# google/speedy

Hardware: AMD Instinct MI355X
Metric: Msamples/s processed (16 kHz mono, 3.5x nonlinear) (higher is better)
Workload: dtype int16 samples; f64 DFT, f32 features, int32 AMDF/OLA

## Files before the change

### include/speedy_hip.h

```cpp
#ifndef SPEEDY_HIP_H_
#define SPEEDY_HIP_H_
#include <stddef.h>
#include <stdint.h>
#ifdef __cplusplus
extern "C" {
#endif

#ifndef SPX_FEATURE_COUNT
#define SPX_FEATURE_COUNT 15
#endif

typedef struct spx_plan* spx_plan_t;

typedef struct {
  int64_t in_off;
  int64_t n_in;
  int64_t out_off;
  int64_t out_cap;
  int32_t channels;
  float speed;
  float nonlinear;
  float feedback;
} spx_stream_job;

// ... 63 lines not shown
int64_t spx_pipeline_submit(spx_pipeline_t p, const int16_t* in, int in_is_device);
int64_t spx_pipeline_submit_jobs(spx_pipeline_t p, const spx_stream_job* jobs, const int16_t* in, int in_is_device);
int spx_pipeline_jobs_fit(spx_pipeline_t p, const spx_stream_job* jobs);
int spx_pipeline_input_consumed(spx_pipeline_t p, int64_t ticket);
int spx_pipeline_wait(spx_pipeline_t p, int64_t ticket, const int16_t** out, const int64_t** offsets, const int64_t** counts);

float* spx_pipeline_host_input_float(spx_pipeline_t p);
int64_t spx_pipeline_submit_float(spx_pipeline_t p, const float* in, int in_is_device);
int64_t spx_pipeline_submit_jobs_float(spx_pipeline_t p, const spx_stream_job* jobs, const float* in, int in_is_device);
int spx_pipeline_wait_float(spx_pipeline_t p, int64_t ticket, const float** out, const int64_t** offsets, const int64_t** counts);

void* spx_host_alloc(size_t bytes);
void spx_host_free(void* p);

int spx_batch_analyze(spx_plan_t plan, const spx_stream_job* jobs, int n_streams, const int16_t* in,
                      void* workspace, size_t workspace_bytes, const spx_taps* taps, void* hip_stream);
int spx_batch_walk(spx_plan_t plan, const spx_stream_job* jobs, int n_streams, const int16_t* in,
                   int16_t* out, int64_t* n_out, void* workspace, size_t workspace_bytes,
                   const spx_taps* taps, void* hip_stream);

size_t spx_batch_workspace_bytes_mixed(const spx_plan_t* plans, int n_plans, const spx_stream_job* jobs,
                                       const int* plan_index, int n_streams);
int spx_batch_run_mixed(const spx_plan_t* plans, int n_plans, const spx_stream_job* jobs, const int* plan_index,
                        int n_streams, const int16_t* in, int16_t* out, int64_t* n_out, void* workspace,
                        size_t workspace_bytes, void* hip_stream);

int spx_batch_run_mixed_taps(const spx_plan_t* plans, int n_plans, const spx_stream_job* jobs, const int* plan_index,
                             int n_streams, const int16_t* in, int16_t* out, int64_t* n_out, void* workspace,
                             size_t workspace_bytes, const spx_taps* taps, void* hip_stream);
int spx_batch_run_mixed_ahead(const spx_plan_t* plans, int n_plans, const spx_stream_job* jobs, const int* plan_index,
                              int n_streams, const int16_t* in, int16_t* out, int64_t* n_out, void* workspace,
                              size_t workspace_bytes, void* hip_stream);

void spx_set_timing(int enabled);
void spx_set_pipeline_chunks(int chunks);
void spx_set_concurrent(int on);
int spx_timing_collect(double* sum_ms_analyze, double* sum_ms_walk, int* n_calls);
const char* spx_batch_kernel_names(spx_plan_t plan, int n_streams, int max_channels, int speedup_only);
const char* spx_batch_kernel_names_lean(spx_plan_t plan, int n_streams, int max_channels, int speedup_only);
int spx_debug_last_walk_form(void);
int spx_debug_kernel_vgprs(int which);
int spx_debug_walk_info(int sample_rate, int channels, int n_streams, int speedup_only, int short_jobs, int lean, int* out5);
int spx_debug_analysis_info(int sample_rate, int* out4);
int spx_debug_lane_consts(int sample_rate, void* out, double* tw, double* tw2, float* win);
int spx_debug_mode_resources(int sample_rate, int channels, int n_streams, int speedup_only, long long* out22);
long long spx_debug_fdiv_check(unsigned seed, unsigned denominators, int exp_lo, int exp_hi);
long long spx_debug_xfade_check(int n_lo, int n_hi);
long long spx_debug_arith_check(unsigned seed, unsigned threads, unsigned per_thread);
int spx_debug_select_check(const unsigned* d, int n_vectors, int p0, int n_lags, int max_period, int two_per_lane, int* lag_index,
                           unsigned* kmin);
int spx_debug_select_fold_check(const unsigned* d, int n_vectors, int p0, int n_lags, int want_max, int fresh, int* out3);
int spx_debug_log_check(unsigned first_block, unsigned end_block, unsigned long long* sums);
int spx_debug_last_call_concurrent(void);
double spx_timing_last_tension_ms(void);
double spx_timing_last_rate_ms(void);

int spx_batch_read_steps(spx_plan_t plan, const spx_stream_job* jobs, int n_streams, const void* workspace,
                         int32_t* steps, void* hip_stream);
int spx_batch_read_steps_mixed(const spx_plan_t* plans, int n_plans, const spx_stream_job* jobs, const int* plan_index,
                               int n_streams, const void* workspace, int32_t* steps, void* hip_stream);

void* spx_device_alloc(size_t bytes);
void spx_device_free(void* p);
int spx_batch_pack_outputs(const spx_stream_job* jobs, int n_streams, const int16_t* out, const int64_t* n_out,
                           int16_t* packed, int64_t* offsets, void* hip_stream);
int spx_copy_to_device(void* dst, const void* src, size_t bytes, void* hip_stream);
int spx_copy_to_host(void* dst, const void* src, size_t bytes, void* hip_stream);
int spx_stream_synchronize(void* hip_stream);

#ifdef __cplusplus
}
#endif
#endif
```

### speedy_amd/_lib.py

```python
import ctypes as C
import os
import subprocess

_HERE = os.path.dirname(os.path.abspath(__file__))
LIB_PATH = os.environ.get("SPEEDY_HIP_LIB") or os.path.join(_HERE, "lib", "libspeedy_hip.so")
_LIB = None

c_short_p = C.POINTER(C.c_short)
c_float_p = C.POINTER(C.c_float)
c_int64_p = C.POINTER(C.c_int64)


class StreamJob(C.Structure):
    _fields_ = [("in_off", C.c_int64), ("n_in", C.c_int64), ("out_off", C.c_int64), ("out_cap", C.c_int64),
                ("channels", C.c_int32), ("speed", C.c_float), ("nonlinear", C.c_float), ("feedback", C.c_float)]


class Taps(C.Structure):
    _fields_ = [("tension", C.c_void_p), ("speed", C.c_void_p), ("features", C.c_void_p),
                ("spectrogram", C.c_void_p), ("normalized", C.c_void_p)]


TENSION_FN = C.CFUNCTYPE(None, C.c_void_p, C.c_int, C.c_float)
FEATURES_FN = C.CFUNCTYPE(None, C.c_void_p, C.c_int, c_float_p)
# ... 4 lines not shown
    "spx_plan_create": (C.c_void_p, [C.c_int, C.c_int]),
    "spx_plan_destroy": (None, [C.c_void_p]),
    "spx_plan_frame_step": (C.c_int, [C.c_void_p]),
    "spx_plan_window_size": (C.c_int, [C.c_void_p]),
    "spx_plan_fft_size": (C.c_int, [C.c_void_p]),
    "spx_plan_future": (C.c_int, [C.c_void_p]),
    "spx_plan_max_required": (C.c_int, [C.c_void_p]),
    "spx_plan_frames": (C.c_int64, [C.c_void_p, C.c_int64]),
    "spx_plan_out_capacity": (C.c_int64, [C.c_void_p, C.c_int64, C.c_float]),
    "spx_plan_out_capacity_for": (C.c_int64, [C.c_void_p, C.c_int64, C.c_float, C.c_float]),
    "spx_batch_workspace_bytes": (C.c_size_t, [C.c_void_p, C.POINTER(StreamJob), C.c_int]),
    "spx_batch_run": (C.c_int, [C.c_void_p, C.POINTER(StreamJob), C.c_int, C.c_void_p, C.c_void_p, C.c_void_p,
                                C.c_void_p, C.c_size_t, C.POINTER(Taps), C.c_void_p]),
    "spx_batch_run_rate": (C.c_int, [C.c_void_p, C.POINTER(StreamJob), c_float_p, C.c_int, C.c_void_p, C.c_void_p, C.c_void_p,
                                     C.c_void_p, C.c_size_t, C.POINTER(Taps), C.c_void_p]),
    "spx_batch_workspace_bytes_rate": (C.c_size_t, [C.c_void_p, C.POINTER(StreamJob), c_float_p, C.c_int]),
    "spx_plan_out_capacity_rate": (C.c_int64, [C.c_void_p, C.c_int64, C.c_float, C.c_float, C.c_float]),
    "spx_batch_workspace_bytes_float": (C.c_size_t, [C.c_void_p, C.POINTER(StreamJob), c_float_p, C.c_int]),
    "spx_batch_run_float": (C.c_int, [C.c_void_p, C.POINTER(StreamJob), c_float_p, C.c_int, C.c_void_p, C.c_void_p, C.c_void_p,
                                      C.c_void_p, C.c_size_t, C.POINTER(Taps), C.c_void_p]),
    "spx_float_to_short": (C.c_int, [C.c_void_p, C.c_void_p, C.c_size_t, C.c_int, C.c_void_p]),
    "spx_short_to_float": (C.c_int, [C.c_void_p, C.c_void_p, C.c_size_t, C.c_void_p]),
    "spx_batch_run_ahead": (C.c_int, [C.c_void_p, C.POINTER(StreamJob), C.c_int, C.c_void_p, C.c_void_p, C.c_void_p,
                                      C.c_void_p, C.c_size_t, C.POINTER(Taps), C.c_void_p]),
    "spx_batch_run_overlapped": (C.c_int, [C.c_void_p, C.POINTER(StreamJob), C.c_int, C.c_void_p, C.c_void_p, C.c_void_p,
                                           C.c_void_p, C.c_size_t, C.POINTER(Taps), C.c_void_p]),
    "spx_batch_run_ahead_when": (C.c_int, [C.c_void_p, C.POINTER(StreamJob), C.c_int, C.c_void_p, C.c_void_p, C.c_void_p,
                                           C.c_void_p, C.c_size_t, C.POINTER(Taps), C.c_void_p, C.c_void_p]),
    "spx_batch_workspace_bytes_mixed": (C.c_size_t, [C.POINTER(C.c_void_p), C.c_int, C.POINTER(StreamJob), C.POINTER(C.c_int), C.c_int]),
    "spx_batch_run_mixed": (C.c_int, [C.POINTER(C.c_void_p), C.c_int, C.POINTER(StreamJob), C.POINTER(C.c_int), C.c_int,
                                      C.c_void_p, C.c_void_p, C.c_void_p, C.c_void_p, C.c_size_t, C.c_void_p]),
    "spx_batch_run_mixed_ahead": (C.c_int, [C.POINTER(C.c_void_p), C.c_int, C.POINTER(StreamJob), C.POINTER(C.c_int), C.c_int,
                                      C.c_void_p, C.c_void_p, C.c_void_p, C.c_void_p, C.c_size_t, C.c_void_p]),
    "spx_batch_run_mixed_taps": (C.c_int, [C.POINTER(C.c_void_p), C.c_int, C.POINTER(StreamJob), C.POINTER(C.c_int), C.c_int,
                                           C.c_void_p, C.c_void_p, C.c_void_p, C.c_void_p, C.c_size_t, C.POINTER(Taps), C.c_void_p]),
    "spx_batch_read_steps": (C.c_int, [C.c_void_p, C.POINTER(StreamJob), C.c_int, C.c_void_p, C.POINTER(C.c_int32), C.c_void_p]),
    "spx_batch_read_steps_mixed": (C.c_int, [C.POINTER(C.c_void_p), C.c_int, C.POINTER(StreamJob), C.POINTER(C.c_int), C.c_int,
                                             C.c_void_p, C.POINTER(C.c_int32), C.c_void_p]),
    "spx_batch_analyze": (C.c_int, [C.c_void_p, C.POINTER(StreamJob), C.c_int, C.c_void_p, C.c_void_p,
                                    C.c_size_t, C.POINTER(Taps), C.c_void_p]),
    "spx_batch_walk": (C.c_int, [C.c_void_p, C.POINTER(StreamJob), C.c_int, C.c_void_p, C.c_void_p, C.c_void_p,
                                 C.c_void_p, C.c_size_t, C.POINTER(Taps), C.c_void_p]),
    "spx_set_timing": (None, [C.c_int]),
    "spx_set_pipeline_chunks": (None, [C.c_int]),
    "spx_set_concurrent": (None, [C.c_int]),
    "spx_timing_collect": (C.c_int, [C.POINTER(C.c_double), C.POINTER(C.c_double), C.POINTER(C.c_int)]),
    "spx_timing_last_tension_ms": (C.c_double, []),
    "spx_timing_last_rate_ms": (C.c_double, []),
    "spx_batch_kernel_names": (C.c_char_p, [C.c_void_p, C.c_int, C.c_int, C.c_int]),
    "spx_batch_kernel_names_lean": (C.c_char_p, [C.c_void_p, C.c_int, C.c_int, C.c_int]),
    "spx_debug_last_walk_form": (C.c_int, []),
    "spx_debug_kernel_vgprs": (C.c_int, [C.c_int]),
    "spx_debug_last_call_concurrent": (C.c_int, []),
    "spx_debug_fdiv_check": (C.c_longlong, [C.c_uint, C.c_uint, C.c_int, C.c_int]),
    "spx_debug_xfade_check": (C.c_longlong, [C.c_int, C.c_int]),
    "spx_debug_select_check": (C.c_int, [C.POINTER(C.c_uint), C.c_int, C.c_int, C.c_int, C.c_int, C.c_int, C.POINTER(C.c_int), C.POINTER(C.c_uint)]),
    "spx_debug_select_fold_check": (C.c_int, [C.POINTER(C.c_uint), C.c_int, C.c_int, C.c_int, C.c_int, C.c_int, C.POINTER(C.c_int)]),
    "spx_debug_arith_check": (C.c_longlong, [C.c_uint, C.c_uint, C.c_uint]),
    "spx_debug_log_check": (C.c_int, [C.c_uint, C.c_uint, C.POINTER(C.c_ulonglong)]),
    "spx_debug_walk_info": (C.c_int, [C.c_int, C.c_int, C.c_int, C.c_int, C.c_int, C.c_int, C.POINTER(C.c_int)]),
    "spx_debug_analysis_info": (C.c_int, [C.c_int, C.POINTER(C.c_int)]),
    "spx_debug_lane_consts": (C.c_int, [C.c_int, C.c_void_p, C.POINTER(C.c_double), C.POINTER(C.c_double), c_float_p]),
    "spx_debug_mode_resources": (C.c_int, [C.c_int, C.c_int, C.c_int, C.c_int, C.POINTER(C.c_longlong)]),
    "spx_pipeline_create": (C.c_void_p, [C.c_void_p, C.POINTER(StreamJob), C.c_int, C.c_int, C.c_uint]),
    "spx_pipeline_create_mixed": (C.c_void_p, [C.POINTER(C.c_void_p), C.c_int, C.POINTER(StreamJob), C.POINTER(C.c_int), C.c_int, C.c_int, C.c_uint]),
    "spx_pipeline_destroy": (None, [C.c_void_p]),
    "spx_pipeline_depth": (C.c_int, [C.c_void_p]),
    "spx_pipeline_input_values": (C.c_size_t, [C.c_void_p]),
    "spx_pipeline_host_input": (C.c_void_p, [C.c_void_p]),
    "spx_pipeline_submit": (C.c_int64, [C.c_void_p, C.c_void_p, C.c_int]),
    "spx_pipeline_submit_jobs": (C.c_int64, [C.c_void_p, C.POINTER(StreamJob), C.c_void_p, C.c_int]),
    "spx_pipeline_jobs_fit": (C.c_int, [C.c_void_p, C.POINTER(StreamJob)]),
    "spx_pipeline_input_consumed": (C.c_int, [C.c_void_p, C.c_int64]),
    "spx_pipeline_wait": (C.c_int, [C.c_void_p, C.c_int64, C.POINTER(C.c_void_p), C.POINTER(C.c_void_p), C.POINTER(C.c_void_p)]),
    "spx_pipeline_host_input_float": (C.c_void_p, [C.c_void_p]),
    "spx_pipeline_submit_float": (C.c_int64, [C.c_void_p, C.c_void_p, C.c_int]),
    "spx_pipeline_submit_jobs_float": (C.c_int64, [C.c_void_p, C.POINTER(StreamJob), C.c_void_p, C.c_int]),
    "spx_pipeline_wait_float": (C.c_int, [C.c_void_p, C.c_int64, C.POINTER(C.c_void_p), C.POINTER(C.c_void_p), C.POINTER(C.c_void_p)]),
    "spx_host_alloc": (C.c_void_p, [C.c_size_t]),
    "spx_host_free": (None, [C.c_void_p]),
    "spx_device_alloc": (C.c_void_p, [C.c_size_t]),
    "spx_device_free": (None, [C.c_void_p]),
    "spx_copy_to_device": (C.c_int, [C.c_void_p, C.c_void_p, C.c_size_t, C.c_void_p]),
    "spx_copy_to_host": (C.c_int, [C.c_void_p, C.c_void_p, C.c_size_t, C.c_void_p]),
    "spx_batch_pack_outputs": (C.c_int, [C.c_void_p, C.c_int, C.c_void_p, C.c_void_p, C.c_void_p, C.c_void_p, C.c_void_p]),
    "spx_stream_synchronize": (C.c_int, [C.c_void_p]),
    "sonicCreateStream": (C.c_void_p, [C.c_int, C.c_int]),
    "sonicDestroyStream": (None, [C.c_void_p]),
    "sonicWriteShortToStream": (C.c_int, [C.c_void_p, c_short_p, C.c_int]),
    "sonicReadShortFromStream": (C.c_int, [C.c_void_p, c_short_p, C.c_int]),
    "sonicWriteFloatToStream": (C.c_int, [C.c_void_p, c_float_p, C.c_int]),
    "sonicReadFloatFromStream": (C.c_int, [C.c_void_p, c_float_p, C.c_int]),
    "sonicSetRate": (None, [C.c_void_p, C.c_float]),
    "sonicSetSpeed": (None, [C.c_void_p, C.c_float]),
    "sonicFlushStream": (C.c_int, [C.c_void_p]),
    "sonicEnableNonlinearSpeedup": (None, [C.c_void_p, C.c_float]),
    "sonicSetDurationFeedbackStrength": (None, [C.c_void_p, C.c_float]),
    "getSonicBufferSize": (C.c_int, [C.c_void_p]),
    "sonicSpectrogramSize": (C.c_int, [C.c_void_p]),
    "sonicTensionCallback": (None, [C.c_void_p, TENSION_FN]),
    "getSonicTensionCallback": (C.c_void_p, [C.c_void_p]),
    "sonicSpeedCallback": (None, [C.c_void_p, TENSION_FN]),
    "getSonicSpeedCallback": (C.c_void_p, [C.c_void_p]),
    "sonicFeaturesCallback": (None, [C.c_void_p, FEATURES_FN]),
    "getSonicFeaturesCallback": (C.c_void_p, [C.c_void_p]),
    "sonicSpectrogramCallback": (None, [C.c_void_p, FEATURES_FN]),
# ... 86 lines not shown
```

### speedy_amd/csrc/speedy_api.hip

```cpp
#include <math.h>
#include <string.h>

#include <algorithm>
#include <string>
#include <vector>

#include "../../include/speedy.h"
#include "spx_internal.h"
#include "spx_log.h"

extern "C" const char* speedyHipLastError(void);
void spx_internal_set_api_error(const std::string& msg);
int spx_internal_match_matlab();

#define SPD_KEEP 24

struct speedyStreamStruct {
  const SpxPlanDev* plan = nullptr;
  int device = 0, rate = 0;
  hipStream_t hs = nullptr;
  int64_t origin = 0, cap = 0;
  float* dFrames = nullptr;
  SpxFrameRec* dRec = nullptr;
  float* dScr = nullptr;
// ... 34 lines not shown
                 {reinterpret_cast<void**>(&s->tTension), sizeof(float), 1, nullptr},
                 {reinterpret_cast<void**>(&s->tSpeed), sizeof(float), 1, nullptr},
                 {reinterpret_cast<void**>(&s->tFeatures), sizeof(float), SPX_FEATURE_COUNT, nullptr},
                 {reinterpret_cast<void**>(&s->tSpec), sizeof(float), P.N, nullptr},
                 {reinterpret_cast<void**>(&s->tNorm), sizeof(float), P.W, nullptr}};
  for (Arr& a : arrs) {
    if (hipMallocAsync(&a.np, (size_t)ncap * a.stride * a.elem, s->hs) != hipSuccess) {
      (void)hipGetLastError();
      for (Arr& b : arrs) if (b.np) (void)hipFreeAsync(b.np, s->hs);
      return false;
    }
  }
  for (Arr& a : arrs) {
    unsigned char* np = static_cast<unsigned char*>(a.np);
    unsigned char* op = static_cast<unsigned char*>(*a.p);
    const size_t row = (size_t)a.stride * a.elem;
    (void)hipMemsetAsync(np, 0, (size_t)ncap * row, s->hs);
    if (op && keep_hi > keep_lo) {
      const int64_t n = std::min(keep_hi, s->origin + s->cap) - keep_lo;
      if (n > 0)
        (void)hipMemcpyAsync(np + (size_t)(keep_lo - lo) * row, op + (size_t)(keep_lo - s->origin) * row, (size_t)n * row,
                             hipMemcpyDeviceToDevice, s->hs);
    }
    if (op) (void)hipFreeAsync(op, s->hs);
    *a.p = a.np;
  }
  s->origin = lo;
  s->cap = ncap;
  return true;
}

static bool launch(speedyStream s, bool new_frame, int64_t k_from, int64_t k_to) {
  const SpxPlanDev& P = *s->plan;
  if (!grow(s, s->T + 2)) { spx_internal_set_api_error("speedy: device allocation failed"); return false; }
  SpxStreamDev J;
  memset(&J, 0, sizeof(J));
  J.frame_off = -s->origin;
  J.n_frames = (int32_t)(s->T + (new_frame ? 1 : 0));
  J.frame_begin = (int32_t)s->T;
  J.channels = 1;
  J.flags = (s->started ? 0 : SPX_F_INIT) | SPX_F_TENSION_RANGE | SPX_F_NO_SPEED;
  J.speed = 2.0f; J.nonlinear = 1.0f; J.feedback = 0.0f;
  J.unit_time0 = (s->time0 == 0) ? 1 : 0;
  J.tension_skip = (int32_t)k_from;
  J.tension_to = (int32_t)k_to;
  if (hipMemcpyAsync(s->dJob, &J, sizeof(J), hipMemcpyHostToDevice, s->hs) != hipSuccess) return false;
  const int64_t fo = J.frame_off;
  SpxTapsDev td;
  td.tension = s->tTension - s->origin - fo; td.speed = s->tSpeed - s->origin - fo;
  td.features = s->tFeatures - (s->origin + fo) * SPX_FEATURE_COUNT;
  td.spectrogram = s->tSpec - (s->origin + fo) * P.N; td.normalized = s->tNorm - (s->origin + fo) * P.W;
  if (new_frame)
    spx_launch_analysis_frames(P, s->dJob, 1, s->dFrames - s->origin * P.W, true, s->dRec, td, s->hs);
  spx_launch_tension(P, s->dJob, 1, s->dState, s->dRec, s->dScr, td, nullptr, nullptr, s->hs);
  if (hipGetLastError() != hipSuccess) { spx_internal_set_api_error("speedy: kernel launch failed"); return false; }
  s->started = true;
  return true;
}


struct FirstOrderFilterStruct { float* d; int device; };

__global__ void hk_fof_iterate_kernel(float* f, float input, float* out) {
  if (threadIdx.x != 0) return;
  const float alpha = f[0];
  const float y = (1 - alpha) * input + alpha * f[1];
  f[1] = y;
  *out = y;
}

__global__ void hk_normalize_kernel(const float* s, float* out, int length, float* energy_out) {
  if (threadIdx.x != 0) return;
  float e = 0.0f;
  for (int i = 1; i < length; i++) e += s[i] * s[i];
  const float eps = 2.2204e-16f;
  const float inv = (float)(1.0 / (__builtin_sqrt((double)e) + (double)eps));
  for (int i = 0; i < length; i++) out[i] = s[i] * inv;
  *energy_out = e;
}

__global__ void hk_preemph_kernel(float* x, int n, float prev) {
  if (threadIdx.x != 0) return;
  for (int i = 0; i < n; i++) {
    const float cur = x[i];
    x[i] = (float)(1.0 * (double)cur - 0.97 * (double)prev);
    prev = cur;
  }
}

__device__ inline float hk_slot(const SpxPlanDev& P, const float* scr, int64_t origin, int64_t cap, int64_t time0, int64_t hi,
                                int64_t tau) {
  const int64_t ring = 2 * (int64_t)(P.F + P.Pp + 1);
  if (tau > hi) tau -= ring * ((tau - hi + ring - 1) / ring);
  else tau += ring * ((hi - tau) / ring);
  const int64_t j = tau - time0;
  return (j >= origin && j < origin + cap && j >= 0) ? scr[4 * (j - origin) + 0] : 0.0f;
}
__device__ inline float hk_hysteresis(const SpxPlanDev& P, const float* scr, int64_t origin, int64_t cap, int64_t time0, int64_t hi,
                                      int64_t k) {
  float future_max = 0.0f, past_max = 0.0f;
  for (int i = 0; i <= P.F; i++) {
    float v = hk_slot(P, scr, origin, cap, time0, hi, k + i);
    v *= P.taperF[i];
    if (v > future_max) future_max = v;
  }
  for (int i = 0; i <= P.Pp; i++) {
    float v = hk_slot(P, scr, origin, cap, time0, hi, k - i);
// ... 429 lines not shown
```

### speedy_amd/csrc/spx_diag.hip

```cpp
#include "spx_engine.h"

extern "C" {
static const char* kernel_names(spx_plan_t plan, int n_streams, int max_channels, int speedup_only, bool lean);
const char* spx_batch_kernel_names(spx_plan_t plan, int n_streams, int max_channels, int speedup_only) {
  return kernel_names(plan, n_streams, max_channels, speedup_only, false);
}
const char* spx_batch_kernel_names_lean(spx_plan_t plan, int n_streams, int max_channels, int speedup_only) {
  return kernel_names(plan, n_streams, max_channels, speedup_only, true);
}
static const char* kernel_names(spx_plan_t plan, int n_streams, int max_channels, int speedup_only, bool lean) {
  static thread_local char buf[256];
  const SpxPlanDev& d = plan->dev;
  const SpxWalkConfig c = spx_walk_config(d, {.n_streams = n_streams, .max_channels = max_channels, .speedup_only = speedup_only != 0,
                                              .any_speed = speedup_only == 0, .lean = lean});
  size_t at = 0;
  auto put = [&](const SpxKernelChoice& k) {
    at += snprintf(buf + at, sizeof(buf) - at, "%s<", k.name);
    for (int i = 0; i < k.n_targs; i++) at += snprintf(buf + at, sizeof(buf) - at, i ? ", %d" : "%d", k.targs[i]);
    at += snprintf(buf + at, sizeof(buf) - at, ">");
  };
  put(spx_analysis_select(d.tile_frames, spx_analysis_ct_window(d)));
  at += snprintf(buf + at, sizeof(buf) - at, ";spx_tension_kernel;");
  put(c.kernel);
  return buf;
}

int spx_debug_last_call_concurrent(void) { return g_last_concurrent.load(std::memory_order_relaxed); }
int spx_debug_kernel_vgprs(int which) {
  if (which == 0) return spx_tension_vgprs();
  const int rate = (which == 2 || which == 4) ? 22050 : 16000;
  const SpxPlanDev* P = spx_internal_shared_plan(rate, 0);
  if (!P) return -1;
  switch (which) {
    case 1: return spx_walk_vgprs(*P, {.n_streams = 256, .max_channels = 1, .speedup_only = true}, nullptr);
    case 2: return spx_walk_vgprs(*P, {.n_streams = 256, .max_channels = 1, .speedup_only = true, .lean = true}, nullptr);
    case 3: case 4: return spx_analysis_vgprs(*P);
    case 5: return spx_walk_vgprs(*P, {.n_streams = 256, .max_channels = 2, .speedup_only = true}, nullptr);
    default: return -1;
  }
}

int spx_debug_walk_info(int sample_rate, int channels, int n_streams, int speedup_only, int short_jobs, int lean, int* out) {
  const SpxPlanDev* P = spx_internal_shared_plan(sample_rate, 0);
  if (!P || !out) return -1;
  const SpxWalkConfig c = spx_walk_config(*P, {.n_streams = n_streams, .max_channels = channels, .speedup_only = speedup_only != 0,
                                               .any_speed = speedup_only == 0, .short_jobs = short_jobs != 0, .lean = lean != 0});
  int scratch = -1;
  out[0] = spx_kernel_vgprs(c.kernel.fn, &scratch);
  out[1] = scratch;
  out[2] = (int)c.lds;
  out[3] = c.fast_kernel ? 16 * c.nwm + c.nwc : 0;
  out[4] = c.waves;
  return 0;
}
int spx_debug_analysis_info(int sample_rate, int* out) {
  const SpxPlanDev* P = spx_internal_shared_plan(sample_rate, 0);
  if (!P || !out) return -1;
  int scratch = -1;
  out[0] = spx_analysis_vgprs(*P, &scratch);
  out[1] = scratch;
  out[2] = (int)spx_analysis_lds_bytes(*P, true);
  out[3] = P->dft_waves;
  return 0;
}

void spx_set_timing(int enabled) { g_timing = enabled != 0; }
void spx_set_concurrent(int on) { g_concurrent = on != 0; }
void spx_set_pipeline_chunks(int chunks) { g_chunks_set = true; g_chunks = chunks < 1 ? 1 : (chunks > SPX_MAX_CHUNKS ? SPX_MAX_CHUNKS : chunks); }
static double g_last_tension_ms = 0.0, g_last_rate_ms = 0.0;
double spx_timing_last_tension_ms(void) { return g_last_tension_ms; }
double spx_timing_last_rate_ms(void) { return g_last_rate_ms; }
int spx_timing_collect(double* sum_ms_analyze, double* sum_ms_walk, int* n_calls) {
  std::lock_guard<std::mutex> g(g_tmu);
  double a = 0, w = 0, t = 0, r = 0;
  for (auto& ev : g_ev_pending) {
    HIPCHK(hipEventSynchronize(ev.b));
    float ms = 0;
    HIPCHK(hipEventElapsedTime(&ms, ev.a, ev.b));
    if (ev.kind == 0) a += ms; else if (ev.kind == 1) w += ms; else if (ev.kind == 3) r += ms; else t += ms;
    g_ev_free.push_back(ev.a);
// ... 118 lines not shown
```

### speedy_amd/csrc/spx_internal.h

```cpp
#pragma once
#include <hip/hip_runtime.h>
#include <stdint.h>

#include <stdlib.h>
#include <type_traits>


#define SPX_FAST_MAX_SPEED 1.0e18f

#define SPX_MAX_STAGES 16
#define SPX_WAVE 64
#define SPX_BLOCK 256
#define SPX_FEATURE_COUNT 15

struct SpxPlanDev {
  int rate;
  int B;
  int W;
  int N;
  int F;
  int Pp;
  int nstages;
  int radix[SPX_MAX_STAGES];
  int minPeriod, maxPeriod, maxRequired, skip;
// ... 79 lines not shown
  int tension_first;
  int pad2_;
};

#define SPX_RATE_MAX_CHANNELS 16
struct SpxRateState {
  int64_t tsm_seen;
  int64_t final_n;
  int32_t old_pos, new_pos;
  int32_t has_left;
  int32_t overflow;
  int16_t left[SPX_RATE_MAX_CHANNELS];
};
void spx_launch_rate(SpxRateState* rs, const SpxStreamState* st, const int64_t* tsm_n, const int16_t* tsm, int16_t* fin,
                     int64_t fin_cap, int channels, int old_rate, int new_rate, float rate, int bypass, int flush,
                     hipStream_t hs);

struct SpxRateJob {
  int64_t tsm_off;
  int64_t tsm_cap;
  int64_t fin_off;
  int64_t fin_cap;
  int32_t channels;
  int32_t old_rate, new_rate;
  int32_t bypass;
  float rate;
  int32_t n_blocks;
  int64_t pad_;
};
int spx_rate_batch_blocks(int64_t frames, int channels);
void spx_launch_rate_batch(const SpxRateJob* jobs, int n_streams, int max_blocks, const SpxStreamState* states, const int64_t* tsm_n,
                           const int16_t* tsm_base, int16_t* fin_base, int64_t* n_out, hipStream_t hs);

struct SpxFrameRec {
  float energy;
  float lsd;
};

struct SpxTapsDev {
  float* tension;
  float* speed;
  float* features;
  float* spectrogram;
  float* normalized;
};

void spx_launch_analysis(const SpxPlanDev& P, const SpxStreamDev* streams, int n_streams, int n_tiles,
                         const int16_t* in, SpxFrameRec* rec, SpxTapsDev taps, const int* tile_order, int* tile_flags,
                         bool mono, hipStream_t st);
void spx_launch_analysis_frames(const SpxPlanDev& P, const SpxStreamDev* streams, int n_tiles, const float* frames,
                                bool preemph, SpxFrameRec* rec, SpxTapsDev taps, hipStream_t st);
void spx_launch_tension(const SpxPlanDev& P, const SpxStreamDev* streams, int n_streams, SpxStreamState* states,
                        const SpxFrameRec* rec, float* scratch, SpxTapsDev taps, const int* tile_flags, int* speed_ready,
                        hipStream_t st);
struct SpxKernelChoice {
  const char* name;
  const void* fn;
  int block;
  int n_targs;
  int targs[5];
};
using SpxAnalysisArgs = void(SpxPlanDev, const SpxStreamDev*, int, const int16_t*, SpxFrameRec*, SpxTapsDev, const int*, int*, const float*, int);
using SpxWalkArgs = void(SpxPlanDev, const SpxStreamDev*, const int16_t*, int16_t*, int64_t*, SpxStreamState*, const float*, int, const int*);
using SpxWalkFastArgs = void(SpxPlanDev, const SpxStreamDev*, const int16_t*, int16_t*, int64_t*, SpxStreamState*, const float*, const int*, int);
template <typename F> struct SpxLaunch;
template <typename... P> struct SpxLaunch<void(P...)> {
  static void go(const SpxKernelChoice& k, int grid, size_t lds, hipStream_t st, P... p) {
    void* args[] = {&p...};
    (void)hipLaunchKernel(k.fn, dim3(grid), dim3(k.block), args, lds, st);
  }
};
struct SpxWalkAsk {
  int n_streams = 0;
  int max_channels = 1;
  bool speedup_only = false;
  bool any_speed = false;
  bool short_jobs = false;
  bool lean = false;
  bool short_window = false;
};
void spx_launch_walk(const SpxPlanDev& P, const SpxWalkAsk& ask, const SpxStreamDev* streams, const int16_t* in, int16_t* out,
                     int64_t* n_out, SpxStreamState* states, const float* scratch, const int* speed_ready, size_t lds_min,
                     hipStream_t st);
size_t spx_analysis_lds_bytes(const SpxPlanDev& P, bool mono);
int spx_analysis_ct_window(const SpxPlanDev& P);
void spx_host_dft(int n, const int* radix, int nstages, const double* tw, const double* in, double* out);
size_t spx_walk_lds_bytes(const SpxPlanDev& P, int max_channels, bool speedup_only);
struct SpxWalkConfig {
  int mode;
  bool fast_kernel;
  int nw;
  int nwm, nwc, wcap;
  int waves;
  size_t lds;
  bool slow;
  SpxKernelChoice kernel;
};
SpxWalkConfig spx_walk_config(const SpxPlanDev& P, const SpxWalkAsk& ask);
SpxKernelChoice spx_walk_select(int nw, int mode);
size_t spx_walk_fast_lds_bytes(const SpxPlanDev& P, int wcap);
bool spx_walk_fast_supports(const SpxPlanDev& P, int nwm);
SpxKernelChoice spx_walk_fast_select(const SpxPlanDev& P, int nwm, int nwc, int wcap, int max_channels, bool slow);
SpxKernelChoice spx_analysis_select(int tile_frames, int ct_window);
#define SPX_NOUT_LOST_PRODUCER INT64_MIN
size_t spx_tension_lds_bytes();
int spx_kernel_vgprs(const void* fn, int* scratch_bytes = nullptr);
int spx_tension_vgprs();
int spx_analysis_vgprs(const SpxPlanDev& P, int* scratch_bytes = nullptr);
int spx_walk_vgprs(const SpxPlanDev& P, const SpxWalkAsk& ask, int* scratch_bytes);
void spx_launch_speed_from_tension(SpxStreamState* state, float tension, float Rg, float feedback, float* speed_out,
                                   hipStream_t st);
int spx_analysis_tile_frames();
int spx_analysis_small_tile_frames();
int spx_analysis_tiny_tile_frames();
int spx_analysis_prefers_small_tile(const SpxPlanDev& P);

struct spx_plan;
int64_t spx_internal_out_bound(const SpxPlanDev& P, int64_t n_in, float speed, bool nonlinear);
const SpxPlanDev* spx_internal_shared_plan(int sample_rate, int match_matlab);
bool spx_internal_analysis_fits(const SpxPlanDev& d);
int64_t spx_internal_frames_for(const SpxPlanDev& d, int64_t n_in);
```

### speedy_amd/csrc/spx_tension.hip

```cpp
#include "spx_internal.h"

#define SPX_CH 512
#ifndef SPX_TCH
#define SPX_TCH 16
#endif
#define SPX_TENSION_THREADS 256

__device__ __forceinline__ float iir_wave(const float* sA, float* sB, int n, float a, float b, float y) {
  const int lane = threadIdx.x;
  for (int b0 = 0; b0 < n; b0 += 64) {
    const int m = n - b0 < 64 ? n - b0 : 64;
    const float ax = a * ((lane < m) ? sA[b0 + lane] : 0.0f);
    if (m == 64) {
      if (lane == 0) {
#pragma unroll
        for (int j = 0; j < 64; j++) {
          const float s = __builtin_bit_cast(float, __builtin_amdgcn_readlane(__builtin_bit_cast(int, ax), j));
          y = s + b * y;
          sB[b0 + j] = y;
        }
      }
      y = __builtin_bit_cast(float, __builtin_amdgcn_readfirstlane(__builtin_bit_cast(int, y)));
      continue;
    }
    if (lane == 0) {
#pragma unroll
      for (int j = 0; j < 64; j++) {
        if (j < m) {
          const float s = __builtin_bit_cast(float, __builtin_amdgcn_readlane(__builtin_bit_cast(int, ax), j));
          y = s + b * y;
          sB[b0 + j] = y;
        }
      }
    }
    y = __builtin_bit_cast(float, __builtin_amdgcn_readfirstlane(__builtin_bit_cast(int, y)));
  }
  return y;
}

__global__ void __launch_bounds__(SPX_TENSION_THREADS)
spx_tension_kernel(SpxPlanDev P, const SpxStreamDev* __restrict__ streams, SpxStreamState* __restrict__ states,
                   const SpxFrameRec* __restrict__ rec_base, float* __restrict__ scratch_base, SpxTapsDev taps,
                   const int* tile_flags, int* speed_ready) {
  constexpr int NT = SPX_TENSION_THREADS;
  __shared__ float sA[SPX_CH];
  __shared__ float sB[SPX_CH];
  __shared__ int sWait;
  const int tid = threadIdx.x;
  const SpxStreamDev S = streams[blockIdx.x];
  const int Ttot = S.n_frames, F = P.F, Pp = P.Pp;
  const int t0 = S.unit_time0 ? 0 : 1;
  const float Rg = S.speed, nl = S.nonlinear, fb = S.feedback;
  if (nl == 0.0f) return;

  struct { float lp, lpf, cur_dur, des_dur; int first_k; } Z;
  if (S.flags & SPX_F_INIT) {
    Z.lp = 2.14204f;
    Z.lpf = 123.837f;
    Z.cur_dur = 0.0f; Z.des_dur = 0.0f;
    Z.first_k = -1;
  } else {
    const SpxStreamState& in = states[blockIdx.x];
    Z.lp = in.lp; Z.lpf = in.lpf; Z.cur_dur = in.cur_dur; Z.des_dur = in.des_dur;
    Z.first_k = in.tension_first;
  }
  const SpxFrameRec* rec = rec_base + S.frame_off;
  float* scr = scratch_base + (size_t)S.frame_off * 4;
  const float lowthr = (float)(0.04 * (double)1.41421f);
  float* tfeat = taps.features ? taps.features + (size_t)S.frame_off * SPX_FEATURE_COUNT : nullptr;

  int fa_c = S.frame_begin;
  int wch = SPX_TCH;
  bool ok_all = true;
  for (;;) {
    int T_c = Ttot;
    if (tile_flags != nullptr && Ttot - fa_c > wch) T_c = fa_c + wch;
    const bool last = T_c >= Ttot;
    if (tile_flags != nullptr && T_c > fa_c) {
      const int TF = P.tile_frames;
      const int i0 = (fa_c - S.frame_begin) / TF, i1 = (T_c - S.frame_begin + TF - 1) / TF;
      if (tid == 0) {
        int ok = 1;
        for (int i = i0; i < i1 && ok; i++) {
          unsigned spins = 0;
          while (__hip_atomic_load(&tile_flags[S.first_tile + i], __ATOMIC_RELAXED, __HIP_MEMORY_SCOPE_AGENT) == 0) {
            __builtin_amdgcn_s_sleep(32);
            if (++spins > (1u << 22)) { ok = 0; break; }
          }
        }
        __builtin_amdgcn_fence(__ATOMIC_ACQUIRE, "agent");
        asm volatile("s_waitcnt vmcnt(0)" ::: "memory");
        sWait = ok;
      }
      __syncthreads();
      if (sWait == 0) { ok_all = false; break; }
    }
    const int fa = fa_c, T = T_c;
    int K0 = (fa + t0 >= F) ? fa + t0 - F : 0;
    if (K0 < S.tension_skip) K0 = S.tension_skip;
    int K = (T + t0 >= F) ? T + t0 - F : 0;
    if (S.flags & SPX_F_TENSION_RANGE) {
      K0 = S.tension_skip;
      if (K > S.tension_to) K = S.tension_to;
    }
    if (Z.first_k < 0 && K > K0) Z.first_k = K0;
    const int first_k = Z.first_k;
    if (T > fa || (S.flags & SPX_F_TENSION_RANGE)) {
      float lp = Z.lp;
      for (int c0 = fa; c0 < T; c0 += SPX_CH) {
        const int n = min(SPX_CH, T - c0);
        for (int i = tid; i < n; i += NT) sA[i] = rec[c0 + i].energy;
        __syncthreads();
        if (tid < 64) lp = iir_wave(sA, sB, n, P.one_minus_alpha, P.alpha, lp);
        __syncthreads();
        for (int i = tid; i < n; i += NT) {
          const float e = sA[i], l = sB[i];
          const float local = e / l;
          const float comp = (float)__builtin_sqrt(local > 2 ? 2.0 : (double)local);
          const int j = c0 + i;
          scr[4 * j + 0] = comp;
          const int k = j + t0 - F;
          if (tfeat && k >= 0) {
            float* f = tfeat + (size_t)k * SPX_FEATURE_COUNT;
            f[1] = l; f[2] = local; f[3] = comp; f[12] = (float)(j + t0);
          }
        }
        if (n > 0) lp = sB[n - 1];
        __syncthreads();
      }
      Z.lp = lp;
      for (int k = K0 + tid; k < K; k += NT) {
        float future_max = 0.0f, past_max = 0.0f;
        for (int i = 0; i <= F; i++) {
          const int tau = k + i;
          float v = (tau >= t0) ? scr[4 * (tau - t0) + 0] : 0.0f;
          v *= P.taperF[i];
          if (v > future_max) future_max = v;
        }
        for (int i = 0; i <= Pp; i++) {
          const int tau = k - i;
          float v = (tau >= t0) ? scr[4 * (tau - t0) + 0] : 0.0f;
          v *= P.taperP[i];
          if (v > past_max) past_max = v;
        }
        const float hyst = (float)((double)(past_max + future_max) / 2.0);
        const float e_cur = (k < t0) ? 0.0f : rec[k - t0].energy;
        const bool low = e_cur <= lowthr || k == first_k;
        const float lsd = low ? 0.0f : rec[k - t0].lsd;
        const float ewld = low ? 0.0f : lsd * hyst;
        scr[4 * k + 1] = hyst;
        scr[4 * k + 2] = ewld;
        if (tfeat) {
          float* f = tfeat + (size_t)k * SPX_FEATURE_COUNT;
          f[0] = e_cur; f[4] = hyst; f[5] = low ? 1.0f : 0.0f; f[6] = lsd; f[7] = ewld;
          f[13] = (float)k; f[14] = lowthr;
        }
      }
      __syncthreads();
      float lpf = Z.lpf;
      for (int c0 = K0; c0 < K; c0 += SPX_CH) {
// ... 64 lines not shown
              if (tid < m) sB[b0 + tid] = req * nl + Rg * (1 - nl);
            }
            if (tid == 0) { sA[0] = cur_dur; sA[1] = des_dur; }
          }
        } else if (tid == 0) {
          for (int i = 0; i < n; i++) {
            float req = sA[i];
            if (fb > 0) {
              const float excess = cur_dur - des_dur;
              req = (float)((double)req + fmax(0.01, (double)(fb * excess)));
            }
            cur_dur += fd / req;
            des_dur += fd / Rg;
            sB[i] = req * nl + Rg * (1 - nl);
          }
          sA[0] = cur_dur;
          sA[1] = des_dur;
        }
        __syncthreads();
        cur_dur = sA[0];
        des_dur = sA[1];
        for (int i = tid; i < n; i += NT) {
          scr[4 * (c0 + i) + 3] = sB[i];
          if (taps.speed) taps.speed[S.frame_off + c0 + i] = sB[i];
        }
        __syncthreads();
      }
      Z.cur_dur = cur_dur;
      Z.des_dur = des_dur;
    }
    if (speed_ready != nullptr) {
      asm volatile("s_waitcnt vmcnt(0)" ::: "memory");
      __syncthreads();
      if (tid == 0) {
        __builtin_amdgcn_fence(__ATOMIC_RELEASE, "agent");
        asm volatile("s_waitcnt vmcnt(0)" ::: "memory");
        __hip_atomic_store(&speed_ready[blockIdx.x], K, __ATOMIC_RELAXED, __HIP_MEMORY_SCOPE_AGENT);
      }
    } else {
      __syncthreads();
    }
    fa_c = T_c;
    if (last) break;
  }
  if (!ok_all && speed_ready != nullptr && tid == 0)
    __hip_atomic_store(&speed_ready[blockIdx.x], -1, __ATOMIC_RELAXED, __HIP_MEMORY_SCOPE_AGENT);
  if (tid == 0) {
    SpxStreamState& o = states[blockIdx.x];
    o.lp = Z.lp; o.lpf = Z.lpf; o.cur_dur = Z.cur_dur; o.des_dur = Z.des_dur;
    o.tension_first = Z.first_k;
  }
}

size_t spx_tension_lds_bytes() { return sizeof(float) * 2 * SPX_CH + 64; }
int spx_tension_vgprs() {
  return spx_kernel_vgprs(reinterpret_cast<const void*>(spx_tension_kernel));
}

__global__ void spx_speed_kernel(SpxStreamState* state, float tension, float Rg, float fb, float* speed_out) {
  if (threadIdx.x != 0) return;
  float v;
  if ((double)Rg > 1.0) {
    v = (float)fmax(1.0, (double)(Rg + (1 - Rg) * tension));
  } else {
    v = (float)fmax(0.01, fmin(1.0, (double)(Rg - (1 - Rg) * tension)));
  }
  float cur_dur = state->cur_dur, des_dur = state->des_dur;
  if (fb > 0) {
    const float excess = cur_dur - des_dur;
    v = (float)((double)v + fmax(0.01, (double)(fb * excess)));
  }
  const float fd = (float)(1.0 / 100.0);
  cur_dur += fd / v;
  des_dur += fd / Rg;
  state->cur_dur = cur_dur;
  state->des_dur = des_dur;
  *speed_out = v;
}
void spx_launch_speed_from_tension(SpxStreamState* state, float tension, float Rg, float feedback, float* speed_out,
                                   hipStream_t st) {
  hipLaunchKernelGGL(spx_speed_kernel, dim3(1), dim3(64), 0, st, state, tension, Rg, feedback, speed_out);
}

void spx_launch_tension(const SpxPlanDev& P, const SpxStreamDev* streams, int n_streams, SpxStreamState* states,
                        const SpxFrameRec* rec, float* scratch, SpxTapsDev taps, const int* tile_flags, int* speed_ready,
                        hipStream_t st) {
  if (n_streams <= 0) return;
  hipLaunchKernelGGL(spx_tension_kernel, dim3(n_streams), dim3(SPX_TENSION_THREADS), 0, st, P, streams, states, rec,
                     scratch, taps, tile_flags, speed_ready);
}
```

Baseline: 49760.

## Fuse tension stages into a single-pass chunked loop with register-held taper weights

Adds a one-pass tension kernel that processes each chunk of frames through compression, hysteresis window, second IIR and speed computation in one loop. This replaces the separate multi-pass sweeps over scratch memory. It keeps a small LDS halo window, prefetches the next chunk's energies and records, and holds the taper weights in lanes that are read with readlane. The old multi-pass kernel is kept for tension-range requests and for F/Pp combinations other than 12/8 and 8/12. This adds code complexity, and correctness depends on the halo and chunk bookkeeping.

Result: no change. 50190, median of 6 (+0.9%).

```diff
diff --git a/include/speedy_hip.h b/include/speedy_hip.h
--- a/include/speedy_hip.h
+++ b/include/speedy_hip.h
@@ -139,6 +139,7 @@
 int spx_debug_select_fold_check(const unsigned* d, int n_vectors, int p0, int n_lags, int want_max, int fresh, int* out3);
 int spx_debug_log_check(unsigned first_block, unsigned end_block, unsigned long long* sums);
 int spx_debug_last_call_concurrent(void);
+int spx_debug_tension_chunk(void);
 double spx_timing_last_tension_ms(void);
 double spx_timing_last_rate_ms(void);
 
diff --git a/speedy_amd/_lib.py b/speedy_amd/_lib.py
--- a/speedy_amd/_lib.py
+++ b/speedy_amd/_lib.py
@@ -80,6 +80,7 @@
     "spx_debug_last_walk_form": (C.c_int, []),
     "spx_debug_kernel_vgprs": (C.c_int, [C.c_int]),
     "spx_debug_last_call_concurrent": (C.c_int, []),
+    "spx_debug_tension_chunk": (C.c_int, []),
     "spx_debug_fdiv_check": (C.c_longlong, [C.c_uint, C.c_uint, C.c_int, C.c_int]),
     "spx_debug_xfade_check": (C.c_longlong, [C.c_int, C.c_int]),
     "spx_debug_select_check": (C.c_int, [C.POINTER(C.c_uint), C.c_int, C.c_int, C.c_int, C.c_int, C.c_int, C.POINTER(C.c_int), C.POINTER(C.c_uint)]),
diff --git a/speedy_amd/csrc/speedy_api.hip b/speedy_amd/csrc/speedy_api.hip
--- a/speedy_amd/csrc/speedy_api.hip
+++ b/speedy_amd/csrc/speedy_api.hip
@@ -110,7 +110,7 @@
   td.spectrogram = s->tSpec - (s->origin + fo) * P.N; td.normalized = s->tNorm - (s->origin + fo) * P.W;
   if (new_frame)
     spx_launch_analysis_frames(P, s->dJob, 1, s->dFrames - s->origin * P.W, true, s->dRec, td, s->hs);
-  spx_launch_tension(P, s->dJob, 1, s->dState, s->dRec, s->dScr, td, nullptr, nullptr, s->hs);
+  spx_launch_tension(P, s->dJob, 1, s->dState, s->dRec, s->dScr, td, nullptr, nullptr, s->hs, true);
   if (hipGetLastError() != hipSuccess) { spx_internal_set_api_error("speedy: kernel launch failed"); return false; }
   s->started = true;
   return true;
diff --git a/speedy_amd/csrc/spx_diag.hip b/speedy_amd/csrc/spx_diag.hip
--- a/speedy_amd/csrc/spx_diag.hip
+++ b/speedy_amd/csrc/spx_diag.hip
@@ -26,6 +26,7 @@
 }
 
 int spx_debug_last_call_concurrent(void) { return g_last_concurrent.load(std::memory_order_relaxed); }
+int spx_debug_tension_chunk(void) { return spx_tension_chunk_frames(); }
 int spx_debug_kernel_vgprs(int which) {
   if (which == 0) return spx_tension_vgprs();
   const int rate = (which == 2 || which == 4) ? 22050 : 16000;
diff --git a/speedy_amd/csrc/spx_internal.h b/speedy_amd/csrc/spx_internal.h
--- a/speedy_amd/csrc/spx_internal.h
+++ b/speedy_amd/csrc/spx_internal.h
@@ -155,7 +155,7 @@
                                 bool preemph, SpxFrameRec* rec, SpxTapsDev taps, hipStream_t st);
 void spx_launch_tension(const SpxPlanDev& P, const SpxStreamDev* streams, int n_streams, SpxStreamState* states,
                         const SpxFrameRec* rec, float* scratch, SpxTapsDev taps, const int* tile_flags, int* speed_ready,
-                        hipStream_t st);
+                        hipStream_t st, bool tension_range = false);
 struct SpxKernelChoice {
   const char* name;
   const void* fn;
@@ -207,6 +207,7 @@
 SpxKernelChoice spx_analysis_select(int tile_frames, int ct_window);
 #define SPX_NOUT_LOST_PRODUCER INT64_MIN
 size_t spx_tension_lds_bytes();
+int spx_tension_chunk_frames();
 int spx_kernel_vgprs(const void* fn, int* scratch_bytes = nullptr);
 int spx_tension_vgprs();
 int spx_analysis_vgprs(const SpxPlanDev& P, int* scratch_bytes = nullptr);
diff --git a/speedy_amd/csrc/spx_tension.hip b/speedy_amd/csrc/spx_tension.hip
--- a/speedy_amd/csrc/spx_tension.hip
+++ b/speedy_amd/csrc/spx_tension.hip
@@ -1,4 +1,5 @@
 #include "spx_internal.h"
+#include "spx_walk_common.h"
 
 #define SPX_CH 512
 #ifndef SPX_TCH
@@ -38,14 +39,195 @@
   return y;
 }
 
-__global__ void __launch_bounds__(SPX_TENSION_THREADS)
-spx_tension_kernel(SpxPlanDev P, const SpxStreamDev* __restrict__ streams, SpxStreamState* __restrict__ states,
-                   const SpxFrameRec* __restrict__ rec_base, float* __restrict__ scratch_base, SpxTapsDev taps,
-                   const int* tile_flags, int* speed_ready) {
+struct SpxTensionCarry { float lp, lpf, cur_dur, des_dur; int first_k; };
+
+#define SPX_TC SPX_TENSION_THREADS
+#define SPX_THALO 20
+
+template <int F, int PP>
+__device__ __forceinline__ void hyst_window(const float* w, float tw, float& future_max, float& past_max) {
+  future_max = 0.0f; past_max = 0.0f;
+#pragma unroll
+  for (int i = 0; i <= F; i++) {
+    float v = w[PP + i];
+    v *= __builtin_bit_cast(float, __builtin_amdgcn_readlane(__builtin_bit_cast(int, tw), i));
+    if (v > future_max) future_max = v;
+  }
+#pragma unroll
+  for (int i = 0; i <= PP; i++) {
+    float v = w[PP - i];
+    v *= __builtin_bit_cast(float, __builtin_amdgcn_readlane(__builtin_bit_cast(int, tw), 32 + i));
+    if (v > past_max) past_max = v;
+  }
+}
+
+__device__ __forceinline__ void tension_one_pass(const SpxPlanDev& P, const SpxStreamDev& S, SpxTensionCarry& Z,
+                                                 const SpxFrameRec* __restrict__ rec, float* __restrict__ scr, float* tfeat,
+                                                 const SpxTapsDev& taps, float* sA, float* sB, float* sW, float* sCarry,
+                                                 int fa, int T, int K0, int K, int t0, float lowthr, float tw) {
+  constexpr int C = SPX_TC;
+  const int tid = threadIdx.x, F = P.F, Pp = P.Pp;
+  const float Rg = S.speed, nl = S.nonlinear, fb = S.feedback;
+  const int first_k = Z.first_k;
+  const bool speeds = !(S.flags & SPX_F_NO_SPEED);
+  const float fd = (float)(1.0 / 100.0);
+  float lp = Z.lp, lpf = Z.lpf, cur_dur = Z.cur_dur, des_dur = Z.des_dur;
+  int kc = K0, nprev = 0;
+  float e_in = (fa + tid < T) ? rec[fa + tid].energy : 0.0f;
+  SpxFrameRec rk = {0.0f, 0.0f};
+  if (kc + tid < K && kc + tid >= t0) rk = rec[kc + tid - t0];
+  for (int p = fa; p < T;) {
+    const int pe = min(T, p + C), np = pe - p;
+    int n = min(K, pe + t0 - F) - kc;
+    if (n < 0) n = 0;
+    const int w0 = kc - Pp - t0;
+    if (tid < np) sA[tid] = e_in;
+    const bool halo = n > 0 && tid < SPX_THALO && w0 + tid < p;
+    float hv = 0.0f;
+    if (halo) {
+      if (nprev > 0) hv = sW[nprev + tid];
+      else if (w0 + tid >= 0) hv = scr[4 * (w0 + tid) + 0];
+    }
+    __syncthreads();
+    if (tid < 64) lp = iir_wave(sA, sB, np, P.one_minus_alpha, P.alpha, lp);
+    __syncthreads();
+    if (tid < np) {
+      const float e = e_in, l = sB[tid];
+      const float local = e / l;
+      const float comp = (float)__builtin_sqrt(local > 2 ? 2.0 : (double)local);
+      const int j = p + tid;
+      scr[4 * j + 0] = comp;
+      if (n > 0 && j >= w0) sW[j - w0] = comp;
+      const int k = j + t0 - F;
+      if (tfeat && k >= 0) {
+        float* f = tfeat + (size_t)k * SPX_FEATURE_COUNT;
+        f[1] = l; f[2] = local; f[3] = comp; f[12] = (float)(j + t0);
+      }
+    }
+    if (halo) sW[tid] = hv;
+    lp = unif(sB[np - 1]);
+    __syncthreads();
+    float e_nx = 0.0f;
+    SpxFrameRec rk_nx = rk;
+    if (n == 0 && pe + tid < T) e_nx = rec[pe + tid].energy;
+    if (n > 0) {
+      const int k = kc + tid;
+      float hyst = 0.0f, ewld = 0.0f;
+      bool low = true;
+      if (tid < n) {
+        float future_max, past_max;
+        if (F == 12) hyst_window<12, 8>(sW + tid, tw, future_max, past_max);
+        else hyst_window<8, 12>(sW + tid, tw, future_max, past_max);
+        hyst = (float)((double)(past_max + future_max) / 2.0);
+        const float e_cur = (k < t0) ? 0.0f : rk.energy;
+        low = e_cur <= lowthr || k == first_k;
+        const float lsd = low ? 0.0f : rk.lsd;
+        ewld = low ? 0.0f : lsd * hyst;
+        scr[4 * k + 1] = hyst;
+        scr[4 * k + 2] = ewld;
+        if (tfeat) {
+          float* f = tfeat + (size_t)k * SPX_FEATURE_COUNT;
+          f[0] = e_cur; f[4] = hyst; f[5] = low ? 1.0f : 0.0f; f[6] = lsd; f[7] = ewld;
+          f[13] = (float)k; f[14] = lowthr;
+        }
+        sA[tid] = ewld;
+      }
+      if (pe + tid < T) e_nx = rec[pe + tid].energy;
+      rk_nx.energy = 0.0f; rk_nx.lsd = 0.0f;
+      if (k + n < K && k + n >= t0) rk_nx = rec[k + n - t0];
+      __syncthreads();
+      if (tid < 64) lpf = iir_wave(sA, sB, n, P.one_minus_alpha, P.alpha, lpf);
+      __syncthreads();
+      if (tid < n) {
+        const float l = sB[tid];
+        float rel = 0.0f, sc = 0.0f;
+        if (!low) {
+          rel = (float)((double)ewld / ((double)l + 0.01 * (double)123.979f));
+          sc = (float)fmin((double)rel, (double)(4 * 0.971975f));
+        }
+        const float a = 0.5f, b = 0.25f, M_E_ = 0.7f, M_S = 1.0f;
+        const float tension = a * (hyst - M_E_) + b * (sc - M_S);
+        float v;
+        if ((double)Rg > 1.0) {
+          v = (float)fmax(1.0, (double)(Rg + (1 - Rg) * tension));
+        } else {
+          v = (float)fmax(0.01, fmin(1.0, (double)(Rg - (1 - Rg) * tension)));
+        }
+        scr[4 * k + 2] = tension;
+        scr[4 * k + 3] = v;
+        if (tfeat) {
+          float* f = tfeat + (size_t)k * SPX_FEATURE_COUNT;
+          f[8] = l; f[9] = rel; f[10] = sc; f[11] = tension;
+        }
+        if (taps.tension) taps.tension[S.frame_off + k] = tension;
+        sA[tid] = v;
+      }
+      lpf = unif(sB[n - 1]);
+      if (speeds) {
+        __syncthreads();
+        if (!(fb > 0)) {
+          if (tid < 64) {
+            const float cstep = fd / Rg;
+            for (int b0 = 0; b0 < n; b0 += 64) {
+              const int m = n - b0 < 64 ? n - b0 : 64;
+              const float req = (tid < m) ? sA[b0 + tid] : 1.0f;
+              const float q = fd / req;
+              if (m == 64) {
+#pragma unroll
+                for (int j = 0; j < 64; j++) {
+                  cur_dur += __builtin_bit_cast(float, __builtin_amdgcn_readlane(__builtin_bit_cast(int, q), j));
+                  des_dur += cstep;
+                }
+              } else {
+#pragma unroll
+                for (int j = 0; j < 64; j++) {
+                  if (j < m) {
+                    cur_dur += __builtin_bit_cast(float, __builtin_amdgcn_readlane(__builtin_bit_cast(int, q), j));
+                    des_dur += cstep;
+                  }
+                }
+              }
+              if (tid < m) sB[b0 + tid] = req * nl + Rg * (1 - nl);
+            }
+            if (tid == 0) { sCarry[0] = cur_dur; sCarry[1] = des_dur; }
+          }
+        } else if (tid == 0) {
+          for (int i = 0; i < n; i++) {
+            float req = sA[i];
+            const float excess = cur_dur - des_dur;
+            req = (float)((double)req + fmax(0.01, (double)(fb * excess)));
+            cur_dur += fd / req;
+            des_dur += fd / Rg;
+            sB[i] = req * nl + Rg * (1 - nl);
+          }
+          sCarry[0] = cur_dur;
+          sCarry[1] = des_dur;
+        }
+        __syncthreads();
+        cur_dur = unif(sCarry[0]);
+        des_dur = unif(sCarry[1]);
+        if (tid < n) {
+          scr[4 * k + 3] = sB[tid];
+          if (taps.speed) taps.speed[S.frame_off + k] = sB[tid];
+        }
+      }
+    }
+    p = pe; kc += n; nprev = n;
+    e_in = e_nx; rk = rk_nx;
+  }
+  Z.lp = lp; Z.lpf = lpf; Z.cur_dur = cur_dur; Z.des_dur = des_dur;
+}
+
+template <bool ONE_PASS>
+__device__ __forceinline__ void tension_body(const SpxPlanDev& P, const SpxStreamDev* __restrict__ streams, SpxStreamState* __restrict__ states,
+                                             const SpxFrameRec* __restrict__ rec_base, float* __restrict__ scratch_base, const SpxTapsDev& taps,
+                                             const int* tile_flags, int* speed_ready) {
   constexpr int NT = SPX_TENSION_THREADS;
-  __shared__ float sA[SPX_CH];
-  __shared__ float sB[SPX_CH];
+  __shared__ float sL[ONE_PASS ? 3 * SPX_TC + SPX_THALO : 2 * SPX_CH];
+  __shared__ float sCarry[2];
   __shared__ int sWait;
+  float* const sA = sL;
+  float* const sB = sL + (ONE_PASS ? SPX_TC : SPX_CH);
   const int tid = threadIdx.x;
   const SpxStreamDev S = streams[blockIdx.x];
   const int Ttot = S.n_frames, F = P.F, Pp = P.Pp;
@@ -53,7 +235,13 @@
   const float Rg = S.speed, nl = S.nonlinear, fb = S.feedback;
   if (nl == 0.0f) return;
 
-  struct { float lp, lpf, cur_dur, des_dur; int first_k; } Z;
+  float tw = 0.0f;
+  if constexpr (ONE_PASS) {
+    const int l = tid & 63;
+    if (l <= F) tw = P.taperF[l];
+    else if (l >= 32 && l - 32 <= Pp) tw = P.taperP[l - 32];
+  }
+  SpxTensionCarry Z;
   if (S.flags & SPX_F_INIT) {
     Z.lp = 2.14204f;
     Z.lpf = 123.837f;
@@ -105,7 +293,9 @@
     }
     if (Z.first_k < 0 && K > K0) Z.first_k = K0;
     const int first_k = Z.first_k;
-    if (T > fa || (S.flags & SPX_F_TENSION_RANGE)) {
+    if constexpr (ONE_PASS) {
+      if (T > fa) tension_one_pass(P, S, Z, rec, scr, tfeat, taps, sA, sB, sL + 2 * SPX_TC, sCarry, fa, T, K0, K, t0, lowthr, tw);
+    } else if (T > fa || (S.flags & SPX_F_TENSION_RANGE)) {
       float lp = Z.lp;
       for (int c0 = fa; c0 < T; c0 += SPX_CH) {
         const int n = min(SPX_CH, T - c0);
@@ -276,9 +466,25 @@
   }
 }
 
+__global__ void __launch_bounds__(SPX_TENSION_THREADS)
+spx_tension_kernel(SpxPlanDev P, const SpxStreamDev* __restrict__ streams, SpxStreamState* __restrict__ states,
+                   const SpxFrameRec* __restrict__ rec_base, float* __restrict__ scratch_base, SpxTapsDev taps,
+                   const int* tile_flags, int* speed_ready) {
+  tension_body<true>(P, streams, states, rec_base, scratch_base, taps, tile_flags, speed_ready);
+}
+__global__ void __launch_bounds__(SPX_TENSION_THREADS)
+spx_tension_passes_kernel(SpxPlanDev P, const SpxStreamDev* __restrict__ streams, SpxStreamState* __restrict__ states,
+                          const SpxFrameRec* __restrict__ rec_base, float* __restrict__ scratch_base, SpxTapsDev taps,
+                          const int* tile_flags, int* speed_ready) {
+  tension_body<false>(P, streams, states, rec_base, scratch_base, taps, tile_flags, speed_ready);
+}
+
 size_t spx_tension_lds_bytes() { return sizeof(float) * 2 * SPX_CH + 64; }
+int spx_tension_chunk_frames() { return SPX_TC; }
 int spx_tension_vgprs() {
-  return spx_kernel_vgprs(reinterpret_cast<const void*>(spx_tension_kernel));
+  const int a = spx_kernel_vgprs(reinterpret_cast<const void*>(spx_tension_kernel));
+  const int b = spx_kernel_vgprs(reinterpret_cast<const void*>(spx_tension_passes_kernel));
+  return a > b ? a : b;
 }
 
 __global__ void spx_speed_kernel(SpxStreamState* state, float tension, float Rg, float fb, float* speed_out) {
@@ -308,8 +514,9 @@
 
 void spx_launch_tension(const SpxPlanDev& P, const SpxStreamDev* streams, int n_streams, SpxStreamState* states,
                         const SpxFrameRec* rec, float* scratch, SpxTapsDev taps, const int* tile_flags, int* speed_ready,
-                        hipStream_t st) {
+                        hipStream_t st, bool tension_range) {
   if (n_streams <= 0) return;
-  hipLaunchKernelGGL(spx_tension_kernel, dim3(n_streams), dim3(SPX_TENSION_THREADS), 0, st, P, streams, states, rec,
+  const bool one_pass = !tension_range && ((P.F == 12 && P.Pp == 8) || (P.F == 8 && P.Pp == 12));
+  hipLaunchKernelGGL(one_pass ? spx_tension_kernel : spx_tension_passes_kernel, dim3(n_streams), dim3(SPX_TENSION_THREADS), 0, st, P, streams, states, rec,
                      scratch, taps, tile_flags, speed_ready);
 }
```
